# zju3dv/OnePose_Plus_Plus

Hardware: AMD Instinct MI355X
Metric: query images/sec (2D-3D match fwd) at 512x512 img x 5k pts (higher is better)
Workload: dtype f32 (operands as exact bf16 triples, f32 accumulate)

## Files before the change

### onepose_plus_plus_amd/csrc/enc_layer64.hip

```cpp
#include <stdlib.h>

#include <type_traits>

#include "enc_frag.h"

namespace {

constexpr int R64 = 64, C = 256, NW = 8, NT = 512, D = 32;
constexpr int SA = a_stride_bytes(C);
constexpr int SS = C + 4;
constexpr int OFF_S = R64 * SA, OFF_Z = OFF_S + 32 * SS * 4;
constexpr size_t kLds64 = OFF_Z + 1024;

__global__ __launch_bounds__(NT) void enc_layer64_kernel(const OppEncChain a) {
  extern __shared__ __attribute__((aligned(16))) char smem[];
  char* A = smem;
  float* S = reinterpret_cast<float*>(smem + OFF_S);
  float* z_sh = reinterpret_cast<float*>(smem + OFF_Z);

  const int tid = threadIdx.x, lane = tid & 63;
  const int wave = __builtin_amdgcn_readfirstlane(tid >> 6);
  const int half = lane >> 5, l31 = lane & 31;

  const int chunks0 = (a.len0 + R64 - 1) / R64;
  const int stream = (int)blockIdx.x >= chunks0 ? 1 : 0;
  const int cidx = stream ? blockIdx.x - chunks0 : blockIdx.x;
  const int seg_len = stream ? a.len1 : a.len0;
  const int row0 = (stream ? a.len0 : 0) + cidx * R64;
  const int nrows = min(R64, seg_len - cidx * R64);
  const float* qrows = (stream && a.q1 != nullptr) ? a.q1 + (size_t)(cidx * R64) * a.ldq : a.q + (size_t)row0 * a.ldq;

  const char* a_lane = A + l31 * SA + half * 48;
  auto gemm = [&](auto ntile_c, auto depth_c, auto s0_c, auto s1_c, auto ks_c, const void* wf, int t0, f32x16 (&acc)[2][decltype(ntile_c)::value], int tstep = 1) {
    constexpr int NTILE = decltype(ntile_c)::value, DEPTH = decltype(depth_c)::value;
    constexpr int S0 = decltype(s0_c)::value, S1 = decltype(s1_c)::value, KS = decltype(ks_c)::value;
    constexpr int NSTEP = S1 - S0;
    const __amdgpu_buffer_rsrc_t rsrc = __builtin_amdgcn_make_buffer_rsrc(const_cast<void*>(wf), 0, 0x7fffffff, 0x00020000);
    const int voff = lane * 16;
    u32x4 bq[DEPTH][NTILE][3];
    u32x4 af[2][2][3];
    auto load_b = [&](int s, int slot) {
#pragma unroll
      for (int j = 0; j < NTILE; ++j)
#pragma unroll
        for (int p = 0; p < 3; ++p)
          bq[slot][j][p] = __builtin_amdgcn_raw_buffer_load_b128(rsrc, voff, (((t0 + j * tstep) * KS + S0 + s) * 3 + p) * 1024, 0);
    };
    auto load_a = [&](int s, int slot) {
#pragma unroll
      for (int i = 0; i < 2; ++i)
#pragma unroll
        for (int q = 0; q < 3; ++q) af[slot][i][q] = *reinterpret_cast<const u32x4*>(a_lane + i * 32 * SA + s * 96 + q * 16);
    };
#pragma unroll
    for (int s = 0; s < DEPTH && s < NSTEP; ++s) load_b(s, s);
    load_a(0, 0);
    __builtin_amdgcn_sched_barrier(0);
    constexpr int PA[6] = {2, 0, 1, 1, 0, 0};
    constexpr int PB[6] = {0, 2, 1, 0, 1, 0};
#pragma unroll
    for (int s = 0; s < NSTEP; ++s) {
      if (s + 1 < NSTEP) load_a(s + 1, (s + 1) & 1);
#pragma unroll
      for (int pr = 0; pr < 6; ++pr)
#pragma unroll
        for (int i = 0; i < 2; ++i)
#pragma unroll
          for (int j = 0; j < NTILE; ++j)
            acc[i][j] = __builtin_amdgcn_mfma_f32_32x32x16_bf16(__builtin_bit_cast(bf16x8, af[s & 1][i][PA[pr]]),
                                                                 __builtin_bit_cast(bf16x8, bq[s % DEPTH][j][PB[pr]]), acc[i][j], 0, 0, 0);
      if (s + DEPTH < NSTEP) load_b(s + DEPTH, s % DEPTH);
      __builtin_amdgcn_sched_barrier(0);
    }
  };
  auto ic = [](auto v) { return v; };
  (void)ic;
  auto stage = [&](const f32x16& t, int col0, bool relu) {
#pragma unroll
    for (int r = 0; r < 16; ++r) {
      const int row = (r & 3) + 8 * (r >> 2) + 4 * half;
      float v = t[r];
      if (relu) v = v < 0.f ? 0.f : v;
      S[row * SS + col0 + l31] = v;
    }
  };
  auto split_staged = [&](int rb, int g0) {
#pragma unroll
    for (int i = 0; i < 32 * (C / 8) / NT; ++i) {
      const int p = tid + i * NT;
      const int r = p / (C / 8), g = p - r * (C / 8);
      const float4* s4 = reinterpret_cast<const float4*>(S + r * SS + g * 8);
      split8_store(s4[0], s4[1], A + (rb + r) * SA + (g0 + g) * 48);
    }
  };
  typedef float vec_t __attribute__((ext_vector_type(4)));
  auto layernorm_rows = [&](const float* gamma, const float* beta, float eps, auto mode_c, int rb) {
    constexpr int MODE = decltype(mode_c)::value;
    const vec_t gmv = *reinterpret_cast<const vec_t*>(gamma + lane * 4);
    const vec_t btv = *reinterpret_cast<const vec_t*>(beta + lane * 4);
    constexpr int RPW = 32 / NW;
    float v[RPW][4], sm[RPW], mean[RPW], rstd[RPW];
#pragma unroll
    for (int r = 0; r < RPW; ++r) {
      const vec_t t = *reinterpret_cast<const vec_t*>(S + (wave * RPW + r) * SS + lane * 4);
      sm[r] = 0.f;
#pragma unroll
      for (int i = 0; i < 4; ++i) {
        v[r][i] = t[i];
        sm[r] += t[i];
      }
    }
#pragma unroll
    for (int r = 0; r < RPW; ++r) sm[r] = opp_wave_sum_dpp(sm[r]);
#pragma unroll
    for (int r = 0; r < RPW; ++r) {
      mean[r] = sm[r] / (float)C;
      sm[r] = 0.f;
#pragma unroll
      for (int i = 0; i < 4; ++i) {
        const float d = v[r][i] - mean[r];
        sm[r] = opp_ln_sq_acc(d, sm[r]);
      }
    }
#pragma unroll
    for (int r = 0; r < RPW; ++r) sm[r] = opp_wave_sum_dpp(sm[r]);
#pragma unroll
    for (int r = 0; r < RPW; ++r) rstd[r] = 1.0f / sqrtf(sm[r] / (float)C + eps);
#pragma unroll
    for (int r = 0; r < RPW; ++r) {
      const int lr = rb + wave * RPW + r;
      float y[4];
#pragma unroll
      for (int i = 0; i < 4; ++i) y[i] = opp_ln_affine(v[r][i], mean[r], rstd[r], gmv[i], btv[i]);
      if constexpr (MODE != 0) {
        if (lr < nrows) {
          const vec_t xr = *reinterpret_cast<const vec_t*>(a.X + (size_t)(row0 + lr) * a.ldx + lane * 4);
          vec_t o;
#pragma unroll
          for (int i = 0; i < 4; ++i) o[i] = xr[i] + y[i];
          *reinterpret_cast<vec_t*>(a.out + (size_t)(row0 + lr) * a.ldo + lane * 4) = o;
#pragma unroll
          for (int i = 0; i < 4; ++i) y[i] = o[i];
        } else {
#pragma unroll
          for (int i = 0; i < 4; ++i) y[i] = 0.f;
        }
      }
      if constexpr (MODE != 1) {
        char* g = A + lr * SA + ((lane * 4) >> 3) * 48 + ((lane * 4) & 7) * 2;
#pragma unroll
        for (int i = 0; i < 4; i += 2) {
          unsigned hi, mid, lo;
          split2(y[i], y[i + 1], hi, mid, lo);
          *reinterpret_cast<unsigned*>(g + i * 2) = hi;
          *reinterpret_cast<unsigned*>(g + 16 + i * 2) = mid;
          *reinterpret_cast<unsigned*>(g + 32 + i * 2) = lo;
        }
      }
    }
  };
  auto zero2 = [](auto& acc) {
#pragma unroll
    for (auto& row : acc)
#pragma unroll
      for (auto& t : row)
#pragma unroll
        for (int r = 0; r < 16; ++r) t[r] = 0.f;
  };
  using I0 = std::integral_constant<int, 0>;
  using I1 = std::integral_constant<int, 1>;
  using I2 = std::integral_constant<int, 2>;
  using I3 = std::integral_constant<int, 3>;
  using I4 = std::integral_constant<int, 4>;
  using I16 = std::integral_constant<int, 16>;
  using I32 = std::integral_constant<int, 32>;

#pragma unroll
  for (int i = 0; i < R64 * (C / 8) / NT; ++i) {
    const int p = tid + i * NT;
    const int r = p / (C / 8), g = p - r * (C / 8);
    float4 v0 = make_float4(0.f, 0.f, 0.f, 0.f), v1 = v0;
    if (r < nrows) {
      const float4* s4 = reinterpret_cast<const float4*>(a.X + (size_t)(row0 + r) * a.ldx + g * 8);
      v0 = s4[0];
      v1 = s4[1];
    }
    split8_store(v0, v1, A + r * SA + g * 48);
  }
  const int src = a.cross ? 1 - stream : stream;
  const float src_len = (float)(src ? a.len1 : a.len0);
  const float* kvp = (src && a.kv1 != nullptr) ? a.kv1 : a.kv + (size_t)src * (C * D);
  const float* ksp = (src && a.ks1 != nullptr) ? a.ks1 : a.ks + (size_t)src * C;
  const int h = wave;
  float bk[16];
#pragma unroll
  for (int i = 0; i < 16; ++i) bk[i] = kvp[(h * D + 2 * i + half) * D + l31];
  __syncthreads();
  f32x16 hid[2][2];
  zero2(hid);
  gemm(I2{}, I3{}, I0{}, I16{}, I32{}, a.w1, wave * 2, hid);
  __syncthreads();

  constexpr int QS = 258;
  float* qsh = S;
#pragma unroll
  for (int rh = 0; rh < 2; ++rh) {
#pragma unroll
    for (int i = 0; i < 32 * (C / 4) / NT; ++i) {
      const int e = tid + i * NT;
      const int r = e / (C / 4), c4 = e - r * (C / 4);
      float4 q = make_float4(0.f, 0.f, 0.f, 0.f);
      if (rh * 32 + r < nrows) q = *reinterpret_cast<const float4*>(qrows + (size_t)(rh * 32 + r) * a.ldq + c4 * 4);
      float2* dst = reinterpret_cast<float2*>(qsh + r * QS + c4 * 4);
      dst[0] = make_float2(q.x, q.y);
      dst[1] = make_float2(q.z, q.w);
    }
    __syncthreads();
    if (tid < 8 * 32) {
      const int tok = tid & 31, hh = tid >> 5;
      const float* q = qsh + tok * QS + hh * D;
      const float* k = ksp + hh * D;
      float den = 0.f;
#pragma unroll
      for (int d = 0; d < D; ++d) den = fmaf(q[d], k[d], den);
      z_sh[hh * 32 + tok] = 1.0f / (den + a.eps_attn);
    }
    f32x16 num;
#pragma unroll
    for (int r = 0; r < 16; ++r) num[r] = 0.f;
#pragma unroll
    for (int i = 0; i < 16; ++i) num = __builtin_amdgcn_mfma_f32_32x32x2f32(qsh[l31 * QS + h * D + 2 * i + half], bk[i], num, 0, 0, 0);
    __syncthreads();
    {
      char* col = A + (h * 4 + (l31 >> 3)) * 48 + (l31 & 7) * 2;
#pragma unroll
      for (int r = 0; r < 16; ++r) {
        const int row = (r & 3) + 8 * (r >> 2) + 4 * half;
        const float v = (num[r] * z_sh[h * 32 + row]) * src_len;
        unsigned hi, mid, lo;
        split2(v, 0.f, hi, mid, lo);
        char* d = col + (rh * 32 + row) * SA;
        *reinterpret_cast<unsigned short*>(d) = (unsigned short)hi;
        *reinterpret_cast<unsigned short*>(d + 16) = (unsigned short)mid;
        *reinterpret_cast<unsigned short*>(d + 32) = (unsigned short)lo;
      }
    }
    __syncthreads();
  }

  {
    f32x16 acc[2][1];
    zero2(acc);
    gemm(I1{}, I4{}, I0{}, I16{}, I16{}, a.wm, wave, acc);
    __syncthreads();
#pragma unroll
    for (int rh = 0; rh < 2; ++rh) {
      stage(acc[rh][0], wave * 32, false);
      __syncthreads();
      layernorm_rows(a.g1, a.b1, a.eps_ln, I0{}, rh * 32);
      __syncthreads();
    }
  }

  gemm(I2{}, I3{}, I16{}, I32{}, I32{}, a.w1, wave * 2, hid);
  __syncthreads();

  f32x16 out[2][1];
  zero2(out);
#pragma unroll
  for (int kh = 0; kh < 2; ++kh) {
#pragma unroll
    for (int rh = 0; rh < 2; ++rh) {
      if (wave / (NW / 2) == kh) {
        const int c0 = (wave - kh * (NW / 2)) * 64;
        stage(hid[rh][0], c0, true);
        stage(hid[rh][1], c0 + 32, true);
      }
      __syncthreads();
      split_staged(rh * 32, 0);
      __syncthreads();
    }
    if (kh == 0) gemm(I1{}, I4{}, I0{}, I16{}, I32{}, a.w2, wave, out);
    else gemm(I1{}, I4{}, I16{}, I32{}, I32{}, a.w2, wave, out);
    __syncthreads();
  }

  const bool fold = a.wq_next != nullptr;
#pragma unroll
  for (int rh = 0; rh < 2; ++rh) {
    stage(out[rh][0], wave * 32, false);
    __syncthreads();
    if (fold) layernorm_rows(a.g2, a.b2, a.eps_ln, I2{}, rh * 32);
    else layernorm_rows(a.g2, a.b2, a.eps_ln, I1{}, rh * 32);
    __syncthreads();
  }
  if (!fold) return;

  float* qdst = (stream && a.qkv_out1 != nullptr) ? a.qkv_out1 + (size_t)(cidx * R64) * (3 * C) : a.qkv_out + (size_t)row0 * (3 * C);
  const float vdiv = (float)seg_len;
  auto finish_qkv = [&](f32x16& t, int rb, bool qk) {
#pragma unroll
    for (int r = 0; r < 16; ++r) {
      const int row = rb + (r & 3) + 8 * (r >> 2) + 4 * half;
      float v = 0.f;
      if (row < nrows) {
        v = t[r];
        if (qk) v = v > 0.f ? v + 1.f : __expf(v);
        else v = v / vdiv;
        if (stream == 0 && a.qmask != nullptr) v *= a.qmask[row0 + row];
      }
      t[r] = v;
    }
  };
  auto store_qkv = [&](const f32x16& t, int rb, int tile) {
    const int col = tile * 32 + l31;
#pragma unroll
    for (int r = 0; r < 16; ++r) {
      const int row = rb + (r & 3) + 8 * (r >> 2) + 4 * half;
      if (row < nrows) qdst[(size_t)row * (3 * C) + col] = t[r];
    }
  };
  const bool kv_fold = a.kv_part != nullptr;
  {
    f32x16 acc[2][1];
    zero2(acc);
    gemm(I1{}, I4{}, I0{}, I16{}, I16{}, a.wq_next, h, acc);
#pragma unroll
    for (int i = 0; i < 2; ++i) {
      finish_qkv(acc[i][0], i * 32, true);
      store_qkv(acc[i][0], i * 32, h);
    }
  }
  f32x16 acc[2][2];
  zero2(acc);
  gemm(I2{}, I3{}, I0{}, I16{}, I16{}, a.wq_next, NW + h, acc, NW);
#pragma unroll
  for (int i = 0; i < 2; ++i) {
    finish_qkv(acc[i][0], i * 32, true);
    finish_qkv(acc[i][1], i * 32, false);
  }
  if (!kv_fold) {
#pragma unroll
    for (int i = 0; i < 2; ++i) {
      store_qkv(acc[i][0], i * 32, NW + h);
      store_qkv(acc[i][1], i * 32, 2 * NW + h);
    }
    return;
  }
  {
    f32x16 kvacc;
#pragma unroll
    for (int r = 0; r < 16; ++r) kvacc[r] = 0.f;
    float ksum = 0.f;
    auto swap = [](float x, float y, float& lo, float& hi) {
      const auto r = __builtin_amdgcn_permlane32_swap(__builtin_bit_cast(unsigned, x), __builtin_bit_cast(unsigned, y), false, false);
      lo = __builtin_bit_cast(float, (unsigned)r[0]);
      hi = __builtin_bit_cast(float, (unsigned)r[1]);
    };
#pragma unroll
    for (int i = 0; i < 2; ++i)
#pragma unroll
      for (int q = 0; q < 4; ++q) {
        float kk[2][2], vv[2][2];
#pragma unroll
        for (int e = 0; e < 2; ++e) {
          swap(acc[i][0][4 * q + 2 * e], acc[i][0][4 * q + 2 * e + 1], kk[0][e], kk[1][e]);
          swap(acc[i][1][4 * q + 2 * e], acc[i][1][4 * q + 2 * e + 1], vv[0][e], vv[1][e]);
        }
#pragma unroll
        for (int g = 0; g < 2; ++g)
#pragma unroll
          for (int e = 0; e < 2; ++e) {
            kvacc = __builtin_amdgcn_mfma_f32_32x32x2f32(kk[g][e], vv[g][e], kvacc, 0, 0, 0);
            ksum += kk[g][e];
          }
      }
    float* kvp = a.kv_part + (size_t)blockIdx.x * (C * D) + h * (D * D);
#pragma unroll
    for (int r = 0; r < 16; ++r) {
      const int d = (r & 3) + 8 * (r >> 2) + 4 * half;
      kvp[d * D + l31] = kvacc[r];
    }
    const float tot = ksum + __shfl_xor(ksum, 32, 64);
    if (half == 0) a.ks_part[(size_t)blockIdx.x * C + h * D + l31] = tot;
  }
}

}

int opp_enc_layer64(const OppEncChain& a, hipStream_t stream) {
  OPP_CHECK_ARG(a.C == 256 && a.apply && a.X && a.out && a.q && a.kv && a.ks && a.wm && a.w1 && a.w2 && a.g1 && a.b1 && a.g2 && a.b2,
                "enc_layer64: coarse level (C = 256) with the fused attention apply only");
  OPP_CHECK_ARG(a.len0 >= 0 && a.len1 >= 0 && a.len0 + a.len1 > 0, "enc_layer64: empty token set");
  auto al16 = [](const void* p) { return (reinterpret_cast<uintptr_t>(p) & 15) == 0; };
  OPP_CHECK_ARG(al16(a.X) && al16(a.out) && al16(a.q) && a.ldx % 4 == 0 && a.ldo % 4 == 0 && a.ldq % 4 == 0 && al16(a.g1) && al16(a.b1) &&
                    al16(a.g2) && al16(a.b2) && al16(a.wm) && al16(a.w1) && al16(a.w2) && al16(a.q1), "enc_layer64: operands must be 16-byte aligned");
  OPP_CHECK_ARG(a.wq_next == nullptr || (a.qkv_out != nullptr && al16(a.wq_next)), "enc_layer64: folded projection needs its output buffer");
  OPP_CHECK_ARG((a.kv_part == nullptr) == (a.ks_part == nullptr) && (a.kv_part == nullptr || (a.wq_next != nullptr && a.qkv_out1 == nullptr)),
                "enc_layer64: the KV partials need the folded projection and both of their buffers");
  static OppLdsOnce lds_once;
  opp_lds_opt_in(reinterpret_cast<const void*>(enc_layer64_kernel), kLds64, lds_once);
  const int tiles = opp_cdiv(a.len0, R64) + opp_cdiv(a.len1, R64);
  OppProfScope prof(OPP_PROF_ENC_CHAIN, stream, 2.0 * (double)(a.len0 + a.len1) * ((a.wq_next ? 10.0 : 7.0) * C * C + 32.0 * C));
  hipLaunchKernelGGL(enc_layer64_kernel, dim3(tiles), dim3(NT), kLds64, stream, a);
  OPP_CHECK_LAUNCH("enc_layer64_kernel");
  return OPP_OK;
}
```

### onepose_plus_plus_amd/csrc/gemm_mfma.hip

```cpp
#include <stdlib.h>

#include <mutex>
#include <type_traits>

#include <vector>

#include "opp_internal.h"

typedef float f32x16 __attribute__((ext_vector_type(16)));
typedef _Float16 f16x8 __attribute__((ext_vector_type(8)));
typedef __bf16 bf16x8 __attribute__((ext_vector_type(8)));
typedef __bf16 bf16x2 __attribute__((ext_vector_type(2)));
typedef float f32x2 __attribute__((ext_vector_type(2)));

namespace {

constexpr int lds_stride(int prec) { return prec == OPP_PREC_BF16X3 ? 52 : 36; }

__device__ __forceinline__ void opp_split4_b3(const float4 v, uint2& hi, uint2& mid, uint2& lo) {
  auto lvl = [](float a, float b, float& ra, float& rb) -> unsigned {
    const f32x2 t = {a, b};
    const unsigned p = __builtin_bit_cast(unsigned, __builtin_convertvector(t, bf16x2));
    ra = a - __uint_as_float(p << 16);
    rb = b - __uint_as_float(p & 0xffff0000u);
// ... 1632 lines not shown
        hipLaunchKernelGGL(opp_gemm_kfold_kernel, dim3(opp_cdiv(g.M, 128) * opp_cdiv(g.n_store, 128)), dim3(512), lds, stream, gf);
        OPP_CHECK_LAUNCH("opp_gemm_kfold_kernel");
        return OPP_OK;
      }
      OppGemm gs = g;
      gs.C = g.splitk_ws;
      gs.C3 = nullptr;
      gs.k_splits = kSplits;
      gs.k_chunks_per_split = opp_cdiv(nkc, kSplits);
      gs.split_stride = (size_t)g.M * g.ldc;
      gs.bias = nullptr;
      gs.res_mode = OPP_RES_NONE;
      gs.R = nullptr;
      gs.act = OPP_ACT_NONE;
      gs.splitk_ws = nullptr;
      OPP_TRY(opp_gemm_launch_cfg(gs, 25, stream));
      const size_t n4 = (size_t)g.M * g.ldc / 4;
      const int blocks = (int)((n4 + 255) / 256 < 2048 ? (n4 + 255) / 256 : 2048);
      OppProfScope prof_epi(OPP_PROF_SPLITK_EPILOGUE, stream, (double)(kSplits + 1 + (g.res_mode == OPP_RES_DIRECT ? 1 : 0)) * (double)g.M * g.ldc * 4.0);
      hipLaunchKernelGGL(splitk_epilogue_kernel, dim3(blocks), dim3(256), 0, stream, reinterpret_cast<const float4*>(g.splitk_ws), kSplits, n4, n4, g.ldc / 4,
                         reinterpret_cast<const float4*>(g.bias), g.res_mode == OPP_RES_DIRECT ? reinterpret_cast<const float4*>(g.R) : nullptr, g.act,
                         reinterpret_cast<float4*>(g.C), g.C3, g.ld3);
      OPP_CHECK_LAUNCH("splitk_epilogue_kernel");
      return OPP_OK;
    }
  }
  const bool auto_cfg = cfg < 0;
  if (cfg < 0) cfg = choose_tile(g);
  OPP_CHECK_ARG(g.stat_rowmax == nullptr || (g.prec == OPP_PREC_BF16X3 ? (cfg == 25 || cfg == 20) : cfg == 0),
                "gemm: fused softmax statistics need the 128x128 tile (config 0; bf16x3: config 25, or 20 = 256x128)");
  if (g.ln_gamma != nullptr) {
    if (auto_cfg || (cfg != 30 && cfg != 26)) cfg = g.n_store == 256 ? 30 : 26;
    auto al = [](const void* p) { return (reinterpret_cast<uintptr_t>(p) & 15) == 0; };
    OPP_CHECK_ARG(g.ln_beta && ((cfg == 30 && g.n_store == 256) || (cfg == 26 && g.n_store == 128)) && g.N == g.n_store && !g.bias &&
                      g.act == OPP_ACT_NONE && g.res_mode == OPP_RES_NONE && g.ldc % 4 == 0 && al(g.C) && al(g.ln_gamma) &&
                      al(g.ln_beta) && (!g.ln_res || (al(g.ln_res) && g.ln_ldres % 4 == 0)),
                  "gemm: fused LayerNorm needs a 256- or 128-column output, no bias/activation/residual mode, aligned operands");
  }
  OppProfScope prof_scope(g.conv && g.k_splits > 1 ? (int)OPP_PROF_CONV_SPLITK : opp_prof_gemm_symbol(cfg, g.conv ? 1 : (g.stat_rowmax ? 2 : 0)), stream,
                          g.alg_flops > 0.0 ? g.alg_flops : 2.0 * (double)g.M * (double)g.N * (double)g.K);
  int rc;
  switch (cfg) {
    case 0: rc = launch_cfg<128, 128, 2, 2>(g, stream); break;
    case 1: rc = launch_cfg<64, 128, 2, 2>(g, stream); break;
    case 2: rc = launch_cfg<64, 64, 2, 2>(g, stream); break;
    case 10: rc = launch_cfg<128, 128, 2, 2, 3>(g, stream); break;
    case 11: rc = launch_cfg<128, 128, 2, 2, 4>(g, stream); break;
    case 20: rc = launch_cfg<256, 128, 4, 2>(g, stream); break;
    case 22:
      rc = conv208(g) ? launch_cfg<128, 224, 2, 4>(g, stream) : launch_cfg<128, 256, 2, 4>(g, stream);
      break;
    case 24: rc = launch_cfg<128, 192, 4, 2>(g, stream); break;
    case 25: rc = launch_cfg<128, 128, 4, 2>(g, stream); break;
    case 27:
      if (g.prec != OPP_PREC_BF16X3 || g.n_store > 224 || (g.n_real > 208 && g.n_real != g.n_store)) {
        opp_set_error("gemm: tile config 27 (128 x 224) is a bf16x3 tile for outputs of <= 208 real and <= 224 stored columns");
        rc = OPP_ERR_UNSUPPORTED;
      } else if (g.conv && (g.a_split || g.k_splits > 1)) {
        rc = launch_cfg<128, 256, 2, 4>(g, stream);
      } else if (g.conv) {
        rc = launch_cfg<128, 224, 2, 4>(g, stream);
      } else {
        rc = launch_cfg<128, 224, 4, 2>(g, stream);
      }
      break;
    case 26: rc = launch_cfg<64, 128, 2, 4>(g, stream); break;
    case 30: rc = launch_cfg<64, 256, 2, 4>(g, stream); break;
    default:
#ifdef OPP_TUNING
      rc = launch_tuning_cfg(g, cfg, stream);
#else
      opp_set_error("gemm: unknown tile config %d", cfg);
      rc = OPP_ERR_INVALID;
#endif
      break;
  }
  return rc;
}

extern "C" int opp_debug_timestamps(void* buf) {
#ifdef OPP_TUNING
  g_dbg_ts = static_cast<unsigned long long*>(buf);
  opp_gemm_ss_debug_timestamps(buf, getenv("OPP_SS_TS_MODE") ? atoi(getenv("OPP_SS_TS_MODE")) : 0);
  return OPP_OK;
#else
  (void)buf;
  opp_set_error("opp_debug_timestamps: library built without -DOPP_TUNING");
  return OPP_ERR_UNSUPPORTED;
#endif
}

int opp_gemm_launch(const OppGemm& g, hipStream_t stream) { return opp_gemm_launch_cfg(g, -1, stream); }

int opp_gemm_choose_tile(const OppGemm& g) {
  int cfg = choose_tile(g);
  if (g.conv && g.prec == OPP_PREC_BF16X3 && splitk_by_shape(g) && g.K / 32 >= 4) cfg = 1000 + 25;
  return cfg;
}
```

### onepose_plus_plus_amd/csrc/opp_internal.h

```cpp
#pragma once
#include "opp_common.h"

enum {
  OPP_PROF_FIRST_NON_GEMM = 1000,
  OPP_PROF_LINATTN_KV = 1000,
  OPP_PROF_LINATTN_APPLY = 1001,
  OPP_PROF_CONF = 1002,
  OPP_PROF_FINE = 1003,
  OPP_PROF_LINATTN_SMALL = 1004,
  OPP_PROF_FINE_GATHER = 1005,
  OPP_PROF_FINE_HEAD = 1006,
  OPP_PROF_FOCAL_FWD = 1007,
  OPP_PROF_FOCAL_BWD = 1008,
  OPP_PROF_ENC_CHAIN = 1009,
  OPP_PROF_SCORE_SWEEP1 = 1010,
  OPP_PROF_SCORE_SWEEP2 = 1011,
  OPP_PROF_CONV_WGRAD = 1013,
  OPP_PROF_CONV_SPLITK = 1014,
  OPP_PROF_CONV_TAIL = 1017,
  OPP_PROF_LINATTN_REDUCE = 1016,
  OPP_PROF_SPLITK_EPILOGUE = 1015,
  OPP_PROF_SCORE_SS = 1012,
};
inline int opp_prof_gemm_symbol(int tile_cfg, int kind) { return kind * 256 + tile_cfg; }
struct OppProfScope {
  OppProfScope(int symbol, hipStream_t stream, double work);
  ~OppProfScope();
  OppProfScope(const OppProfScope&) = delete;
  OppProfScope& operator=(const OppProfScope&) = delete;

 private:
  hipStream_t stream_;
  long long slot_ = -1;
};

int opp_layernorm(const float* x, int ldx, const float* gamma, const float* beta, const float* res, int ldres,
                  float* out, int ldo, int rows, int C, float eps, hipStream_t stream);
int opp_linattn_chunks(int seg_len);
int opp_linattn_kv(const float* k, const float* v, int ld, int n_seg, int seg_len, int C, int D, float* kv_out,
                   float* ks_out, float* scratch, hipStream_t stream);
int opp_linattn_apply(const float* q, int ldq, const float* kv, const float* ks, float* out, int ldo, int n_seg,
                      int seg_len, int src_len, int C, int D, float eps, hipStream_t stream);
size_t opp_linattn_pair_scratch_floats(int len0, int len1);
int opp_linattn_kv_pair(const float* qkv, int ld, int len0, int len1, float* kv, float* ks, float* scratch,
                        hipStream_t stream);
void opp_linattn_chunk_parts(float* scratch, int len0, int len1, float** kv_part, float** ks_part);
int opp_linattn_reduce_chunks(int len0, int len1, float* kv, float* ks, float* scratch, hipStream_t stream);
size_t opp_focal_loss_ws_bytes(size_t n);
int opp_focal_loss_fwd(const float* conf, const short* gt, const float* weight, size_t n, float alpha, float gamma, double* sums,
                       void* ws, size_t ws_bytes, hipStream_t stream);
int opp_focal_loss_bwd(const float* conf, const short* gt, const float* weight, size_t n, float alpha, float gamma,
                       const float* scales, float* grad, hipStream_t stream);
int opp_focal_loss_fwd_ex(const float* conf, const void* gt, int gt_kind, const float* weight, const float* mask0, const float* mask1, int N, int L,
                          size_t n, float alpha, float gamma, double* sums, void* ws, size_t ws_bytes, hipStream_t stream);
int opp_focal_loss_bwd_ex(const float* conf, const void* gt, int gt_kind, const float* weight, const float* mask0, const float* mask1, int N, int L,
                          size_t n, float alpha, float gamma, const float* scales, float* grad, hipStream_t stream);
size_t opp_dual_softmax_bwd_ws_bytes(int B, int N, int L);
int opp_dual_softmax_bwd(const float* g, const float* sim, const float* lse_row, const float* lse_col, int B, int N, int L, float* ds,
                         void* ws, size_t ws_bytes, hipStream_t stream);
bool opp_linattn_small_ok(int len0, int len1, int C, int D);
int opp_full_attention_run(const float* qkv, int n_seg, int len0, int len1, int C, int nhead, int cross, int prec, float* msg,
                           hipStream_t stream);
int opp_linattn_small_pair(const float* qkv, int ld, int n_seg, int len0, int len1, int cross, float* out, int ldo, int C, int D,
                           float eps, hipStream_t stream);
int opp_linattn_apply_pair(const float* qkv, int ld, const float* kv, const float* ks, int cross, float* out, int ldo,
                           int len0, int len1, float eps, hipStream_t stream);
struct OppEncChain {
  int C = 256;
  const float* X = nullptr;
  int ldx = 0;
  float* out = nullptr;
  int ldo = 0;
  int len0 = 0, len1 = 0;
  const float* msg = nullptr;
  int ldm = 0;
  int apply = 0;
  const float* q = nullptr;
  int ldq = 0;
  const float* kv = nullptr;
  const float* ks = nullptr;
  const float* q1 = nullptr;
  const float* kv1 = nullptr;
  const float* ks1 = nullptr;
  const void* wq_next = nullptr;
  float* qkv_out = nullptr;
  float* qkv_out1 = nullptr;
  const float* qmask = nullptr;
  float* kv_part = nullptr;
  float* ks_part = nullptr;
  int cross = 0;
  float eps_attn = 1e-6f;
  const void* wm = nullptr;
  const void* w1 = nullptr;
  const void* w2 = nullptr;
  const float *g1 = nullptr, *b1 = nullptr, *g2 = nullptr, *b2 = nullptr;
  float eps_ln = 1e-5f;
};
size_t opp_frag_b3_bytes(int N, int K);
int opp_pack_frag_b3(const float* w, int N, int K, void* out, hipStream_t stream);
bool opp_enc_chain_ok(int C, int nhead, bool apply);
int opp_enc_chain(const OppEncChain& a, hipStream_t stream);
int opp_enc_layer64(const OppEncChain& a, hipStream_t stream);
enum { OPP_SS_STATS = 1, OPP_SS_CONF = 2, OPP_SS_STATS_STORE = 3 };
struct OppGemmSS {
  const void* A = nullptr;
  const void* B = nullptr;
  int lda = 0, ldb = 0;
  int M = 0, N = 0, K = 0;
  int mode = OPP_SS_STATS;
  float out_mul = 1.f, out_div = 1.f;
  const float* row_mask = nullptr;
  float* stat_rowmax = nullptr;
  float* stat_rowsum = nullptr;
  float* stat_colmax = nullptr;
  float* stat_colsum = nullptr;
  const float* rstat_max = nullptr;
  const float* rstat_sum = nullptr;
  const float* cstat_max = nullptr;
  const float* cstat_sum = nullptr;
  float* C = nullptr;
  int ldc = 0;
  float* part_best = nullptr;
  int* part_arg = nullptr;
  int* part_ties = nullptr;
  float* part_rowmax = nullptr;
  int a_bytes = 0, b_bytes = 0, vec_store = 0;
  int delay = 0;
  unsigned long long* dbg_ts = nullptr;
};
void opp_gemm_ss_debug_timestamps(void* buf, int mode);
int opp_gemm_ss_tile_rows();
int opp_gemm_ss_tile_cols();
int opp_gemm_ss(const OppGemmSS& g, hipStream_t stream);
size_t opp_linear_bwd_ws_bytes(int M, int N, int K, int prec);
int opp_linear_bwd(const float* dY, const float* X, const float* W, int M, int N, int K, float* dX, float* dW, int accumulate_dw, int prec,
                   void* ws, size_t ws_bytes, hipStream_t stream);
size_t opp_linattn_train_ws_bytes(int B, int L, int S, int H, int D);
int opp_linattn_train_fwd(const float* q, const float* k, const float* v, const float* q_mask, const float* kv_mask, int B, int L, int S, int H, int D,
                          float eps, float* out, float* kv, float* ks, void* ws, size_t ws_bytes, hipStream_t stream);
int opp_linattn_train_bwd(const float* q, const float* k, const float* v, const float* q_mask, const float* kv_mask, const float* kv, const float* ks,
                          const float* grad_out, int B, int L, int S, int H, int D, float eps, float* gq, float* gk, float* gv, void* ws,
                          size_t ws_bytes, hipStream_t stream);
bool opp_stem_direct_ok(int cout, int prec);
int opp_stem_direct(const float* img, int H, int W, const float* wsplit, const float* bias, float* out, int ldc, hipStream_t stream, void* out3 = nullptr,
                    int ld3 = 0);
size_t opp_conv_tail_weight_floats(int cin_pad, int ks);
int opp_pack_conv_tail(const float* w, const float* scale, int cout, int cin, int ks, int n0, int cin_pad, float* wt, hipStream_t stream);
int opp_conv_tail(const OppGemm& g, const float* wt, int n0, int ncols, hipStream_t stream);
int opp_fold_bn(const float* gamma, const float* beta, const float* mean, const float* var, float eps, int c,
                int c_pad, float* scale, float* shift, hipStream_t stream);
int opp_pack_conv(const float* w, const float* scale, int cout, int cin, int ks, int cout_pad, int cin_pad,
                  float* out, hipStream_t stream);
int opp_pack_stem(const float* w, const float* scale, int cout, float* out, hipStream_t stream);
int opp_stem_im2col(const float* img, int B, int H, int W, float* col, hipStream_t stream);
int opp_h2_split(const float* in, float* out, size_t n, float* scale2, hipStream_t stream);
int opp_b3_split(const float* in, float* out, size_t n, hipStream_t stream);
int opp_add(const float* a, const float* b, float* out, size_t n, hipStream_t stream);
int opp_pack_affine(const float* src, float fill, const float* scale1, float* out, int n, hipStream_t stream);
int opp_add_cat(const float* a, const float* b, size_t na, const float* c, size_t nc, float* out, hipStream_t stream);
int opp_transpose(const float* in, float* out, int batch, int R, int Cc, hipStream_t stream);
size_t opp_bn_train_scratch_bytes(int rows, int ld);
int opp_bn_train(const float* y, int rows, int ld, int C, const float* gamma, const float* beta, float eps, const float* res,
                 int act, float* out, float* stat_out, void* scratch, hipStream_t stream, float* save_mean = nullptr, float* save_invstd = nullptr);
size_t opp_conv_geo_entries(int P);
int opp_conv_geo(int B, int Ho, int Wo, int Hin, int Win, int ks, int stride, int pad, void* geo, hipStream_t stream);
size_t opp_conv_wgrad_ws_bytes(int P, int cout_pad, int cin_pad, int ks);
int opp_conv_wgrad(const float* dY, int ldy, const float* X, int ldx, size_t x_pixels, const void* geo, int P, int Win, int ks, int cout, int cin,
                   float* dW, int accumulate, void* ws, size_t ws_bytes, hipStream_t stream);
int opp_conv_flip_transpose(const float* w, int cout, int cin, int ks, float* out, hipStream_t stream);
int opp_conv_dilate2(const float* dy, int B, int Ho, int Wo, int ld, float* z, hipStream_t stream);
size_t opp_bn_bwd_scratch_bytes(int rows, int ld);
int opp_bn_backward(const float* dy, const float* y, const float* raw, int rows, int ld, int C, int act, const float* gamma, const float* mean,
                    const float* invstd, float* draw, float* dres, float* dgamma, float* dbeta, int accumulate, void* scratch, hipStream_t stream);
int opp_upsample2x_backward(const float* g, int B, int Hr, int Wr, int ld, float* dr, int accumulate, hipStream_t stream);
int opp_ln_forward(const float* x, const float* gamma, const float* beta, const float* res, int rows, int C, float eps, float* y, float* mean,
                   float* rstd, hipStream_t stream);
size_t opp_ln_backward_ws_bytes(int rows, int C);
int opp_ln_backward(const float* g, const float* x, const float* gamma, const float* mean, const float* rstd, int rows, int C, float* dx,
                    float* dgamma, float* dbeta, void* ws, size_t ws_bytes, hipStream_t stream);
size_t opp_lse_ws_bytes(int B, int N, int L);
int opp_dual_softmax_lse(const float* S, int B, int N, int L, float* lse_row, float* lse_col, float* conf, void* ws, size_t ws_bytes,
                         hipStream_t stream);
int opp_fine_gather_batch(const float* feat, int Hf, int Wf, int C, const long long* b_ids, const long long* j_ids, int M, int wc, int stride, int Wwin,
                          float* win, hipStream_t stream);
int opp_fine_scatter_batch(const float* gwin, int B, int Hf, int Wf, int C, const long long* b_ids, const long long* j_ids, int M, int wc, int stride,
// ... 34 lines not shown
```

Baseline: 590.4.

## Prefetch next-stage weight fragments and query rows across barriers in enc_layer64

Splits the fused-layer GEMM helper into an issue phase and a run phase, so the B-fragment ring for the next GEMM is loaded before the current epilogue, layernorm and barriers rather than at the start of that GEMM. Query rows, layernorm parameters, residual rows and mask values are also prefetched into registers ahead of use, and the attention denominator is computed per wave using readlane instead of by a subset of threads. Full-tile specialisations drop per-row bounds checks in the QKV tail. The cost is higher register pressure from the live prefetch rings, plus timestamp instrumentation that is only built in tuning builds.

Result: no change. 590.0 (-0.1%).

```diff
diff --git a/onepose_plus_plus_amd/csrc/enc_layer64.hip b/onepose_plus_plus_amd/csrc/enc_layer64.hip
--- a/onepose_plus_plus_amd/csrc/enc_layer64.hip
+++ b/onepose_plus_plus_amd/csrc/enc_layer64.hip
@@ -10,7 +10,37 @@
 constexpr int SA = a_stride_bytes(C);
 constexpr int SS = C + 4;
 constexpr int OFF_S = R64 * SA, OFF_Z = OFF_S + 32 * SS * 4;
+#ifdef OPP_TUNING
+constexpr int kTsSlots = 64;
+constexpr size_t kLds64 = OFF_Z + 1024 + NW * kTsSlots * 4;
+#define ENC_TS(id)                                                                      \
+  do {                                                                                  \
+    if (ts_on) {                                                                        \
+      __builtin_amdgcn_sched_barrier(0);                                                \
+      unsigned long long ts_now;                                                        \
+      asm volatile("s_memtime %0\n\ts_waitcnt lgkmcnt(0)" : "=s"(ts_now)::"memory");    \
+      if (lane == 0) ts_sh[wave * kTsSlots + (id)] = (unsigned)ts_now - ts0;            \
+      __builtin_amdgcn_sched_barrier(0);                                                \
+    }                                                                                   \
+  } while (0)
+#define ENC_TS_GEMM(id) ts_gemm = (id)
+#define ENC_TS_DUMP()                                                                   \
+  do {                                                                                  \
+    if (ts_on && ts_sh[wave * kTsSlots + lane] != 0u)    \
+      a.dbg_ts[((size_t)blockIdx.x * NW + wave) * kTsSlots + lane] = ts_sh[wave * kTsSlots + lane];   \
+  } while (0)
+#else
 constexpr size_t kLds64 = OFF_Z + 1024;
+#define ENC_TS(id) do { } while (0)
+#define ENC_TS_GEMM(id) do { } while (0)
+#define ENC_TS_DUMP() do { } while (0)
+#endif
+
+template <int DEPTH, int NTILE>
+struct BRing {
+  static constexpr int kDepth = DEPTH, kTiles = NTILE;
+  u32x4 v[DEPTH][NTILE][3];
+};
 
 __global__ __launch_bounds__(NT) void enc_layer64_kernel(const OppEncChain a) {
   extern __shared__ __attribute__((aligned(16))) char smem[];
@@ -21,6 +51,15 @@
   const int tid = threadIdx.x, lane = tid & 63;
   const int wave = __builtin_amdgcn_readfirstlane(tid >> 6);
   const int half = lane >> 5, l31 = lane & 31;
+#ifdef OPP_TUNING
+  unsigned* ts_sh = reinterpret_cast<unsigned*>(smem + OFF_Z + 1024);
+  const bool ts_on = a.dbg_ts != nullptr;
+  unsigned long long ts_entry;
+  asm volatile("s_memtime %0\n\ts_waitcnt lgkmcnt(0)" : "=s"(ts_entry)::"memory");
+  const unsigned ts0 = (unsigned)ts_entry;
+  int ts_gemm = 0;
+  if (ts_on) ts_sh[wave * kTsSlots + lane] = 0u;
+#endif
 
   const int chunks0 = (a.len0 + R64 - 1) / R64;
   const int stream = (int)blockIdx.x >= chunks0 ? 1 : 0;
@@ -31,29 +70,38 @@
   const float* qrows = (stream && a.q1 != nullptr) ? a.q1 + (size_t)(cidx * R64) * a.ldq : a.q + (size_t)row0 * a.ldq;
 
   const char* a_lane = A + l31 * SA + half * 48;
-  auto gemm = [&](auto ntile_c, auto depth_c, auto s0_c, auto s1_c, auto ks_c, const void* wf, int t0, f32x16 (&acc)[2][decltype(ntile_c)::value], int tstep = 1) {
-    constexpr int NTILE = decltype(ntile_c)::value, DEPTH = decltype(depth_c)::value;
-    constexpr int S0 = decltype(s0_c)::value, S1 = decltype(s1_c)::value, KS = decltype(ks_c)::value;
+  const int voff = lane * 16;
+  auto load_b = [&](auto s0_c, auto ks_c, const __amdgpu_buffer_rsrc_t rsrc, int t0, int tstep, int s, auto& slot) {
+    constexpr int S0 = decltype(s0_c)::value, KS = decltype(ks_c)::value;
+    constexpr int NTILE = sizeof(slot) / sizeof(slot[0]);
+#pragma unroll
+    for (int j = 0; j < NTILE; ++j)
+#pragma unroll
+      for (int p = 0; p < 3; ++p)
+        slot[j][p] = __builtin_amdgcn_raw_buffer_load_b128(rsrc, voff, (((t0 + j * tstep) * KS + S0 + s) * 3 + p) * 1024, 0);
+  };
+  auto gemm_issue = [&](auto s0_c, auto ks_c, const void* wf, int t0, auto& ring, int tstep = 1) {
+    constexpr int DEPTH = std::remove_reference_t<decltype(ring)>::kDepth;
+    const __amdgpu_buffer_rsrc_t rsrc = __builtin_amdgcn_make_buffer_rsrc(const_cast<void*>(wf), 0, 0x7fffffff, 0x00020000);
+#pragma unroll
+    for (int s = 0; s < DEPTH; ++s) load_b(s0_c, ks_c, rsrc, t0, tstep, s, ring.v[s]);
+    __builtin_amdgcn_sched_barrier(0);
+  };
+  auto gemm_run = [&](auto s0_c, auto s1_c, auto ks_c, const void* wf, int t0, auto& ring, auto& acc, int tstep = 1) {
+    using Ring = std::remove_reference_t<decltype(ring)>;
+    constexpr int NTILE = Ring::kTiles, DEPTH = Ring::kDepth;
+    constexpr int S0 = decltype(s0_c)::value, S1 = decltype(s1_c)::value;
     constexpr int NSTEP = S1 - S0;
+    static_assert(DEPTH <= NSTEP, "the issue part loads DEPTH steps");
     const __amdgpu_buffer_rsrc_t rsrc = __builtin_amdgcn_make_buffer_rsrc(const_cast<void*>(wf), 0, 0x7fffffff, 0x00020000);
-    const int voff = lane * 16;
-    u32x4 bq[DEPTH][NTILE][3];
+    auto& bq = ring.v;
     u32x4 af[2][2][3];
-    auto load_b = [&](int s, int slot) {
-#pragma unroll
-      for (int j = 0; j < NTILE; ++j)
-#pragma unroll
-        for (int p = 0; p < 3; ++p)
-          bq[slot][j][p] = __builtin_amdgcn_raw_buffer_load_b128(rsrc, voff, (((t0 + j * tstep) * KS + S0 + s) * 3 + p) * 1024, 0);
-    };
     auto load_a = [&](int s, int slot) {
 #pragma unroll
       for (int i = 0; i < 2; ++i)
 #pragma unroll
         for (int q = 0; q < 3; ++q) af[slot][i][q] = *reinterpret_cast<const u32x4*>(a_lane + i * 32 * SA + s * 96 + q * 16);
     };
-#pragma unroll
-    for (int s = 0; s < DEPTH && s < NSTEP; ++s) load_b(s, s);
     load_a(0, 0);
     __builtin_amdgcn_sched_barrier(0);
     constexpr int PA[6] = {2, 0, 1, 1, 0, 0};
@@ -69,9 +117,11 @@
           for (int j = 0; j < NTILE; ++j)
             acc[i][j] = __builtin_amdgcn_mfma_f32_32x32x16_bf16(__builtin_bit_cast(bf16x8, af[s & 1][i][PA[pr]]),
                                                                  __builtin_bit_cast(bf16x8, bq[s % DEPTH][j][PB[pr]]), acc[i][j], 0, 0, 0);
-      if (s + DEPTH < NSTEP) load_b(s + DEPTH, s % DEPTH);
+      if (s + DEPTH < NSTEP) load_b(s0_c, ks_c, rsrc, t0, tstep, s + DEPTH, bq[s % DEPTH]);
       __builtin_amdgcn_sched_barrier(0);
-    }
+      if (s == 0) ENC_TS(ts_gemm);
+    }
+    ENC_TS(ts_gemm + 1);
   };
   auto ic = [](auto v) { return v; };
   (void)ic;
@@ -94,11 +144,11 @@
     }
   };
   typedef float vec_t __attribute__((ext_vector_type(4)));
-  auto layernorm_rows = [&](const float* gamma, const float* beta, float eps, auto mode_c, int rb) {
+  constexpr int RPW = 32 / NW;
+  auto ln_params = [&](const float* p) { return *reinterpret_cast<const vec_t*>(p + lane * 4); };
+  auto ln_x_row = [&](int lr) { return *reinterpret_cast<const vec_t*>(a.X + (size_t)(row0 + min(lr, nrows - 1)) * a.ldx + lane * 4); };
+  auto layernorm_rows = [&](const vec_t gmv, const vec_t btv, float eps, auto mode_c, int rb, const vec_t* xres) {
     constexpr int MODE = decltype(mode_c)::value;
-    const vec_t gmv = *reinterpret_cast<const vec_t*>(gamma + lane * 4);
-    const vec_t btv = *reinterpret_cast<const vec_t*>(beta + lane * 4);
-    constexpr int RPW = 32 / NW;
     float v[RPW][4], sm[RPW], mean[RPW], rstd[RPW];
 #pragma unroll
     for (int r = 0; r < RPW; ++r) {
@@ -134,7 +184,7 @@
       for (int i = 0; i < 4; ++i) y[i] = opp_ln_affine(v[r][i], mean[r], rstd[r], gmv[i], btv[i]);
       if constexpr (MODE != 0) {
         if (lr < nrows) {
-          const vec_t xr = *reinterpret_cast<const vec_t*>(a.X + (size_t)(row0 + lr) * a.ldx + lane * 4);
+          const vec_t xr = xres[r];
           vec_t o;
 #pragma unroll
           for (int i = 0; i < 4; ++i) o[i] = xr[i] + y[i];
@@ -170,23 +220,44 @@
   using I0 = std::integral_constant<int, 0>;
   using I1 = std::integral_constant<int, 1>;
   using I2 = std::integral_constant<int, 2>;
-  using I3 = std::integral_constant<int, 3>;
-  using I4 = std::integral_constant<int, 4>;
   using I16 = std::integral_constant<int, 16>;
   using I32 = std::integral_constant<int, 32>;
 
+  const int last_row = nrows - 1;
+  constexpr int QS = 258;
+  float* qsh = S;
+  auto q_issue = [&](int rh, float4 (&q)[4]) {
+#pragma unroll
+    for (int i = 0; i < 32 * (C / 4) / NT; ++i) {
+      const int e = tid + i * NT;
+      const int r = e / (C / 4), c4 = e - r * (C / 4);
+      q[i] = *reinterpret_cast<const float4*>(qrows + (size_t)min(rh * 32 + r, last_row) * a.ldq + c4 * 4);
+    }
+  };
+  auto q_store = [&](int rh, const float4 (&q)[4], int nr) {
+#pragma unroll
+    for (int i = 0; i < 32 * (C / 4) / NT; ++i) {
+      const int e = tid + i * NT;
+      const int r = e / (C / 4), c4 = e - r * (C / 4);
+      const bool in = rh * 32 + r < nr;
+      float2* dst = reinterpret_cast<float2*>(qsh + r * QS + c4 * 4);
+      dst[0] = make_float2(in ? q[i].x : 0.f, in ? q[i].y : 0.f);
+      dst[1] = make_float2(in ? q[i].z : 0.f, in ? q[i].w : 0.f);
+    }
+  };
+
+  float4 xv[R64 * (C / 8) / NT][2];
 #pragma unroll
   for (int i = 0; i < R64 * (C / 8) / NT; ++i) {
     const int p = tid + i * NT;
     const int r = p / (C / 8), g = p - r * (C / 8);
-    float4 v0 = make_float4(0.f, 0.f, 0.f, 0.f), v1 = v0;
-    if (r < nrows) {
-      const float4* s4 = reinterpret_cast<const float4*>(a.X + (size_t)(row0 + r) * a.ldx + g * 8);
-      v0 = s4[0];
-      v1 = s4[1];
-    }
-    split8_store(v0, v1, A + r * SA + g * 48);
-  }
+    const float4* s4 = reinterpret_cast<const float4*>(a.X + (size_t)(row0 + min(r, last_row)) * a.ldx + g * 8);
+    xv[i][0] = s4[0];
+    xv[i][1] = s4[1];
+  }
+  float4 qv[4];
+  q_issue(0, qv);
+  __builtin_amdgcn_sched_barrier(0);
   const int src = a.cross ? 1 - stream : stream;
   const float src_len = (float)(src ? a.len1 : a.len0);
   const float* kvp = (src && a.kv1 != nullptr) ? a.kv1 : a.kv + (size_t)src * (C * D);
@@ -195,42 +266,53 @@
   float bk[16];
 #pragma unroll
   for (int i = 0; i < 16; ++i) bk[i] = kvp[(h * D + 2 * i + half) * D + l31];
+  const float ksv = ksp[h * D + l31];
+  BRing<3, 2> ring_w1;
+  gemm_issue(I0{}, I32{}, a.w1, wave * 2, ring_w1);
+  int nrows_sel = nrows;
+  asm volatile("" : "+s"(nrows_sel)::"memory");
+  __builtin_amdgcn_sched_barrier(0);
+#pragma unroll
+  for (int i = 0; i < R64 * (C / 8) / NT; ++i) {
+    const int p = tid + i * NT;
+    const int r = p / (C / 8), g = p - r * (C / 8);
+    const float4 z4 = make_float4(0.f, 0.f, 0.f, 0.f);
+    split8_store(r < nrows_sel ? xv[i][0] : z4, r < nrows_sel ? xv[i][1] : z4, A + r * SA + g * 48);
+  }
+  q_store(0, qv, nrows_sel);
+  ENC_TS(1);
   __syncthreads();
+  ENC_TS(2);
   f32x16 hid[2][2];
   zero2(hid);
-  gemm(I2{}, I3{}, I0{}, I16{}, I32{}, a.w1, wave * 2, hid);
+  ENC_TS_GEMM(3);
+  gemm_run(I0{}, I16{}, I32{}, a.w1, wave * 2, ring_w1, hid);
   __syncthreads();
-
-  constexpr int QS = 258;
-  float* qsh = S;
+  ENC_TS(5);
+
+  BRing<4, 1> ring_c;
+  q_issue(1, qv);
+  gemm_issue(I0{}, I16{}, a.wm, wave, ring_c);
 #pragma unroll
   for (int rh = 0; rh < 2; ++rh) {
-#pragma unroll
-    for (int i = 0; i < 32 * (C / 4) / NT; ++i) {
-      const int e = tid + i * NT;
-      const int r = e / (C / 4), c4 = e - r * (C / 4);
-      float4 q = make_float4(0.f, 0.f, 0.f, 0.f);
-      if (rh * 32 + r < nrows) q = *reinterpret_cast<const float4*>(qrows + (size_t)(rh * 32 + r) * a.ldq + c4 * 4);
-      float2* dst = reinterpret_cast<float2*>(qsh + r * QS + c4 * 4);
-      dst[0] = make_float2(q.x, q.y);
-      dst[1] = make_float2(q.z, q.w);
-    }
+    ENC_TS(6 + 6 * rh);
+    ENC_TS(7 + 6 * rh);
+    {
+      const float* q = qsh + l31 * QS + h * D;
+      float den = 0.f;
+#pragma unroll
+      for (int d = 0; d < D; ++d)
+        den = fmaf(q[d], __builtin_bit_cast(float, __builtin_amdgcn_readlane(__builtin_bit_cast(int, ksv), d)), den);
+      z_sh[h * 32 + l31] = 1.0f / (den + a.eps_attn);
+    }
+    f32x16 num;
+#pragma unroll
+    for (int r = 0; r < 16; ++r) num[r] = 0.f;
+#pragma unroll
+    for (int i = 0; i < 16; ++i) num = __builtin_amdgcn_mfma_f32_32x32x2f32(qsh[l31 * QS + h * D + 2 * i + half], bk[i], num, 0, 0, 0);
+    ENC_TS(8 + 6 * rh);
     __syncthreads();
-    if (tid < 8 * 32) {
-      const int tok = tid & 31, hh = tid >> 5;
-      const float* q = qsh + tok * QS + hh * D;
-      const float* k = ksp + hh * D;
-      float den = 0.f;
-#pragma unroll
-      for (int d = 0; d < D; ++d) den = fmaf(q[d], k[d], den);
-      z_sh[hh * 32 + tok] = 1.0f / (den + a.eps_attn);
-    }
-    f32x16 num;
-#pragma unroll
-    for (int r = 0; r < 16; ++r) num[r] = 0.f;
-#pragma unroll
-    for (int i = 0; i < 16; ++i) num = __builtin_amdgcn_mfma_f32_32x32x2f32(qsh[l31 * QS + h * D + 2 * i + half], bk[i], num, 0, 0, 0);
-    __syncthreads();
+    ENC_TS(9 + 6 * rh);
     {
       char* col = A + (h * 4 + (l31 >> 3)) * 48 + (l31 & 7) * 2;
 #pragma unroll
@@ -245,28 +327,46 @@
         *reinterpret_cast<unsigned short*>(d + 32) = (unsigned short)lo;
       }
     }
+    if (rh == 0) q_store(1, qv, nrows);
+    ENC_TS(10 + 6 * rh);
     __syncthreads();
-  }
-
+    ENC_TS(11 + 6 * rh);
+  }
+
+  BRing<3, 2> ring_w1b;
   {
+    const vec_t g1v = ln_params(a.g1), b1v = ln_params(a.b1);
     f32x16 acc[2][1];
     zero2(acc);
-    gemm(I1{}, I4{}, I0{}, I16{}, I16{}, a.wm, wave, acc);
+    ENC_TS_GEMM(18);
+    gemm_run(I0{}, I16{}, I16{}, a.wm, wave, ring_c, acc);
+    gemm_issue(I16{}, I32{}, a.w1, wave * 2, ring_w1b);
     __syncthreads();
+    ENC_TS(20);
 #pragma unroll
     for (int rh = 0; rh < 2; ++rh) {
       stage(acc[rh][0], wave * 32, false);
       __syncthreads();
-      layernorm_rows(a.g1, a.b1, a.eps_ln, I0{}, rh * 32);
+      ENC_TS(21 + 3 * rh);
+      layernorm_rows(g1v, b1v, a.eps_ln, I0{}, rh * 32, nullptr);
+      ENC_TS(22 + 3 * rh);
       __syncthreads();
-    }
-  }
-
-  gemm(I2{}, I3{}, I16{}, I32{}, I32{}, a.w1, wave * 2, hid);
+      ENC_TS(23 + 3 * rh);
+    }
+  }
+
+  ENC_TS_GEMM(27);
+  gemm_run(I16{}, I32{}, I32{}, a.w1, wave * 2, ring_w1b, hid);
+  gemm_issue(I0{}, I32{}, a.w2, wave, ring_c);
   __syncthreads();
-
+  ENC_TS(29);
+
+  const bool fold = a.wq_next != nullptr;
   f32x16 out[2][1];
   zero2(out);
+  vec_t g2v, b2v, xres[2][RPW];
+  const bool has_mask = fold && stream == 0 && a.qmask != nullptr;
+  float mval = 1.f;
 #pragma unroll
   for (int kh = 0; kh < 2; ++kh) {
 #pragma unroll
@@ -277,74 +377,118 @@
         stage(hid[rh][1], c0 + 32, true);
       }
       __syncthreads();
+      ENC_TS(30 + 7 * kh + 2 * rh);
       split_staged(rh * 32, 0);
       __syncthreads();
-    }
-    if (kh == 0) gemm(I1{}, I4{}, I0{}, I16{}, I32{}, a.w2, wave, out);
-    else gemm(I1{}, I4{}, I16{}, I32{}, I32{}, a.w2, wave, out);
+      ENC_TS(31 + 7 * kh + 2 * rh);
+    }
+    ENC_TS_GEMM(34 + 7 * kh);
+    if (kh == 0) {
+      gemm_run(I0{}, I16{}, I32{}, a.w2, wave, ring_c, out);
+      gemm_issue(I16{}, I32{}, a.w2, wave, ring_c);
+      g2v = ln_params(a.g2);
+      b2v = ln_params(a.b2);
+      if (has_mask) mval = a.qmask[row0 + min(lane, last_row)];
+#pragma unroll
+      for (int i = 2 * RPW - 1; i > 0; --i) xres[i / RPW][i % RPW] = ln_x_row((i / RPW) * 32 + wave * RPW + i % RPW);
+      __builtin_amdgcn_sched_barrier(0);
+      xres[0][0] = ln_x_row(wave * RPW);
+      __builtin_amdgcn_sched_barrier(0);
+    } else {
+      gemm_run(I16{}, I32{}, I32{}, a.w2, wave, ring_c, out);
+      if (fold) gemm_issue(I0{}, I16{}, a.wq_next, h, ring_c);
+    }
     __syncthreads();
-  }
-
-  const bool fold = a.wq_next != nullptr;
+    ENC_TS(36 + 7 * kh);
+  }
+
 #pragma unroll
   for (int rh = 0; rh < 2; ++rh) {
     stage(out[rh][0], wave * 32, false);
     __syncthreads();
-    if (fold) layernorm_rows(a.g2, a.b2, a.eps_ln, I2{}, rh * 32);
-    else layernorm_rows(a.g2, a.b2, a.eps_ln, I1{}, rh * 32);
+    ENC_TS(44 + 3 * rh);
+    if (fold) layernorm_rows(g2v, b2v, a.eps_ln, I2{}, rh * 32, xres[rh]);
+    else layernorm_rows(g2v, b2v, a.eps_ln, I1{}, rh * 32, xres[rh]);
+    ENC_TS(45 + 3 * rh);
     __syncthreads();
-  }
-  if (!fold) return;
+    ENC_TS(46 + 3 * rh);
+  }
+  if (!fold) {
+    ENC_TS_DUMP();
+    return;
+  }
 
   float* qdst = (stream && a.qkv_out1 != nullptr) ? a.qkv_out1 + (size_t)(cidx * R64) * (3 * C) : a.qkv_out + (size_t)row0 * (3 * C);
   const float vdiv = (float)seg_len;
-  auto finish_qkv = [&](f32x16& t, int rb, bool qk) {
+  auto finish_qkv = [&](f32x16& t, int rb, bool qk, auto full_c) {
+    constexpr bool FULL = decltype(full_c)::value;
 #pragma unroll
     for (int r = 0; r < 16; ++r) {
       const int row = rb + (r & 3) + 8 * (r >> 2) + 4 * half;
+      float m = 1.f;
+      if (has_mask) m = __shfl(mval, row, 64);
       float v = 0.f;
-      if (row < nrows) {
+      if (FULL || row < nrows) {
         v = t[r];
         if (qk) v = v > 0.f ? v + 1.f : __expf(v);
         else v = v / vdiv;
-        if (stream == 0 && a.qmask != nullptr) v *= a.qmask[row0 + row];
+        if (has_mask) v *= m;
       }
       t[r] = v;
     }
   };
-  auto store_qkv = [&](const f32x16& t, int rb, int tile) {
+  auto store_qkv = [&](const f32x16& t, int rb, int tile, auto full_c) {
+    constexpr bool FULL = decltype(full_c)::value;
     const int col = tile * 32 + l31;
 #pragma unroll
     for (int r = 0; r < 16; ++r) {
       const int row = rb + (r & 3) + 8 * (r >> 2) + 4 * half;
-      if (row < nrows) qdst[(size_t)row * (3 * C) + col] = t[r];
+      if (FULL || row < nrows) qdst[(size_t)row * (3 * C) + col] = t[r];
     }
   };
   const bool kv_fold = a.kv_part != nullptr;
+  const bool full_tile = nrows == R64;
+  BRing<3, 2> ring_kv;
   {
     f32x16 acc[2][1];
     zero2(acc);
-    gemm(I1{}, I4{}, I0{}, I16{}, I16{}, a.wq_next, h, acc);
-#pragma unroll
-    for (int i = 0; i < 2; ++i) {
-      finish_qkv(acc[i][0], i * 32, true);
-      store_qkv(acc[i][0], i * 32, h);
-    }
+    ENC_TS_GEMM(50);
+    gemm_run(I0{}, I16{}, I16{}, a.wq_next, h, ring_c, acc);
+    gemm_issue(I0{}, I16{}, a.wq_next, NW + h, ring_kv, NW);
+    auto tail = [&](auto full_c) {
+#pragma unroll
+      for (int i = 0; i < 2; ++i) {
+        finish_qkv(acc[i][0], i * 32, true, full_c);
+        store_qkv(acc[i][0], i * 32, h, full_c);
+      }
+    };
+    if (full_tile) tail(std::true_type{});
+    else tail(std::false_type{});
+    ENC_TS(52);
   }
   f32x16 acc[2][2];
   zero2(acc);
-  gemm(I2{}, I3{}, I0{}, I16{}, I16{}, a.wq_next, NW + h, acc, NW);
-#pragma unroll
-  for (int i = 0; i < 2; ++i) {
-    finish_qkv(acc[i][0], i * 32, true);
-    finish_qkv(acc[i][1], i * 32, false);
-  }
+  ENC_TS_GEMM(53);
+  gemm_run(I0{}, I16{}, I16{}, a.wq_next, NW + h, ring_kv, acc, NW);
+  auto tail_kv = [&](auto full_c) {
+#pragma unroll
+    for (int i = 0; i < 2; ++i) {
+      finish_qkv(acc[i][0], i * 32, true, full_c);
+      finish_qkv(acc[i][1], i * 32, false, full_c);
+    }
+    if (!kv_fold) {
+#pragma unroll
+      for (int i = 0; i < 2; ++i) {
+        store_qkv(acc[i][0], i * 32, NW + h, full_c);
+        store_qkv(acc[i][1], i * 32, 2 * NW + h, full_c);
+      }
+    }
+  };
+  if (full_tile) tail_kv(std::true_type{});
+  else tail_kv(std::false_type{});
+  ENC_TS(55);
   if (!kv_fold) {
-#pragma unroll
-    for (int i = 0; i < 2; ++i) {
-      store_qkv(acc[i][0], i * 32, NW + h);
-      store_qkv(acc[i][1], i * 32, 2 * NW + h);
-    }
+    ENC_TS_DUMP();
     return;
   }
   {
@@ -384,11 +528,35 @@
     const float tot = ksum + __shfl_xor(ksum, 32, 64);
     if (half == 0) a.ks_part[(size_t)blockIdx.x * C + h * D + l31] = tot;
   }
+  ENC_TS(56);
+  ENC_TS_DUMP();
 }
 
 }
 
-int opp_enc_layer64(const OppEncChain& a, hipStream_t stream) {
+#ifdef OPP_TUNING
+namespace {
+unsigned* g_enc_ts = nullptr;
+int g_enc_ts_tiles = 0;
+}
+#endif
+void opp_enc_layer64_debug_timestamps(void* buf, int max_tiles) {
+#ifdef OPP_TUNING
+  g_enc_ts = static_cast<unsigned*>(buf);
+  g_enc_ts_tiles = max_tiles;
+#else
+  (void)buf;
+  (void)max_tiles;
+#endif
+}
+
+int opp_enc_layer64(const OppEncChain& a_in, hipStream_t stream) {
+#ifdef OPP_TUNING
+  OppEncChain a = a_in;
+  a.dbg_ts = (opp_cdiv(a.len0, R64) + opp_cdiv(a.len1, R64) <= g_enc_ts_tiles) ? g_enc_ts : nullptr;
+#else
+  const OppEncChain& a = a_in;
+#endif
   OPP_CHECK_ARG(a.C == 256 && a.apply && a.X && a.out && a.q && a.kv && a.ks && a.wm && a.w1 && a.w2 && a.g1 && a.b1 && a.g2 && a.b2,
                 "enc_layer64: coarse level (C = 256) with the fused attention apply only");
   OPP_CHECK_ARG(a.len0 >= 0 && a.len1 >= 0 && a.len0 + a.len1 > 0, "enc_layer64: empty token set");
diff --git a/onepose_plus_plus_amd/csrc/gemm_mfma.hip b/onepose_plus_plus_amd/csrc/gemm_mfma.hip
--- a/onepose_plus_plus_amd/csrc/gemm_mfma.hip
+++ b/onepose_plus_plus_amd/csrc/gemm_mfma.hip
@@ -1738,6 +1738,7 @@
 #ifdef OPP_TUNING
   g_dbg_ts = static_cast<unsigned long long*>(buf);
   opp_gemm_ss_debug_timestamps(buf, getenv("OPP_SS_TS_MODE") ? atoi(getenv("OPP_SS_TS_MODE")) : 0);
+  opp_enc_layer64_debug_timestamps(getenv("OPP_ENC_TS") ? buf : nullptr, getenv("OPP_ENC_TS") ? atoi(getenv("OPP_ENC_TS")) : 0);
   return OPP_OK;
 #else
   (void)buf;
diff --git a/onepose_plus_plus_amd/csrc/opp_internal.h b/onepose_plus_plus_amd/csrc/opp_internal.h
--- a/onepose_plus_plus_amd/csrc/opp_internal.h
+++ b/onepose_plus_plus_amd/csrc/opp_internal.h
@@ -95,12 +95,14 @@
   const void* w2 = nullptr;
   const float *g1 = nullptr, *b1 = nullptr, *g2 = nullptr, *b2 = nullptr;
   float eps_ln = 1e-5f;
+  unsigned* dbg_ts = nullptr;
 };
 size_t opp_frag_b3_bytes(int N, int K);
 int opp_pack_frag_b3(const float* w, int N, int K, void* out, hipStream_t stream);
 bool opp_enc_chain_ok(int C, int nhead, bool apply);
 int opp_enc_chain(const OppEncChain& a, hipStream_t stream);
 int opp_enc_layer64(const OppEncChain& a, hipStream_t stream);
+void opp_enc_layer64_debug_timestamps(void* buf, int max_tiles);
 enum { OPP_SS_STATS = 1, OPP_SS_CONF = 2, OPP_SS_STATS_STORE = 3 };
 struct OppGemmSS {
   const void* A = nullptr;
```
